# alexfrom0815/IR-BPP

Measured on AMD Instinct MI355X. Metric: env steps/sec (placements/sec) across N parallel bins, higher is better.
Workload: dtype f64

## Files before the change

include/irbpp.h:

```cpp
#ifndef IRBPP_H
#define IRBPP_H

#include <stdint.h>

#ifdef __cplusplus
extern "C" {
#endif

typedef struct irbpp_env irbpp_env;

typedef enum {
    IRBPP_OK = 0,
    IRBPP_ERR_ARG = -1,
    IRBPP_ERR_HIP = -2,
    IRBPP_ERR_STATE = -3,
    IRBPP_ERR_DEVICE = -4,
    IRBPP_ERR_NOMEM = -5
} irbpp_status;

typedef struct {
    int32_t num_bins;
    int32_t n_rot;
    int32_t selected;
    int32_t buffer_size;
// ... 13 lines not shown

#define IRBPP_TUNE_NO_BLOCK_PATH  1
#define IRBPP_TUNE_WIDE_KERNEL    2
#define IRBPP_TUNE_NARROW_KERNEL  4
#define IRBPP_TUNE_NO_BOX_PATH    8
#define IRBPP_TUNE_NO_ITEM_ORDER 16
#define IRBPP_TUNE_TRACE_CPW64   32
#define IRBPP_TUNE_TRACE_CPW32   64
#define IRBPP_TUNE_TRACE_CPW16  128
#define IRBPP_TUNE_INLINE_POLYGON 256
#define IRBPP_TUNE_NO_HEAVY_FIRST 512
#define IRBPP_TUNE_FUSED_APPLY 2048
#define IRBPP_TUNE_SPLIT_APPLY 4096
#define IRBPP_TUNE_BLOCK_EMIT 8192
#define IRBPP_TUNE_WAVE_EMIT 16384
#define IRBPP_TUNE_GRAPH 32768
#define IRBPP_TUNE_WG512 65536
#define IRBPP_TUNE_NO_WG512 131072
#define IRBPP_TUNE_TRACE_REFILL 262144
#define IRBPP_TUNE_NO_MIXED_PATH 524288
#define IRBPP_TUNE_CHAIN 1048576
#define IRBPP_TUNE_WG128 2097152
#define IRBPP_TUNE_RECT 4194304
#define IRBPP_TUNE_NO_SPECIALISED 1024

typedef struct {
    double*  reward_dev;
    uint8_t* done_dev;
    int32_t* counter_dev;
    double*  ratio_dev;
    double*  ep_reward_dev;
    int32_t* ep_len_dev;
    uint8_t* stable_dev;
    int32_t* err_dev;
} irbpp_step_out;

const char* irbpp_status_string(int status);
int irbpp_version(void);
const char* irbpp_source_hash(void);

int irbpp_create(const irbpp_config* cfg, irbpp_env** out);
int irbpp_destroy(irbpp_env* env);

int irbpp_load_shapes(irbpp_env* env, int32_t n_shapes,
                      const double* extents, const double* volumes,
                      const int32_t* dims, const int64_t* offsets, int64_t pool_len,
// ... 143 lines not shown
```

irbpp_amd/_lib.py:

```python
from __future__ import annotations

import ctypes as C
import os

from .build import LIB_PATH

c_i32_p = C.POINTER(C.c_int32)
c_f64_p = C.POINTER(C.c_double)


class IrbppConfig(C.Structure):
    _fields_ = [
        ("num_bins", C.c_int32), ("n_rot", C.c_int32), ("selected", C.c_int32), ("buffer_size", C.c_int32),
        ("resolution_a", C.c_double), ("resolution_h", C.c_double), ("resolution_z", C.c_double),
        ("bin", C.c_double * 3), ("scale_z", C.c_double),
        ("traj_start", C.c_int32), ("global_offset", C.c_int32), ("global_bins", C.c_int32),
        ("device", C.c_int32), ("stability", C.c_int32), ("tuning", C.c_int32), ("item_stream", C.c_int32),
    ]


TUNE_NO_BLOCK_PATH, TUNE_WIDE_KERNEL, TUNE_NARROW_KERNEL, TUNE_NO_BOX_PATH, TUNE_NO_ITEM_ORDER = 1, 2, 4, 8, 16
TUNE_TRACE_CPW64, TUNE_TRACE_CPW32, TUNE_TRACE_CPW16, TUNE_INLINE_POLYGON, TUNE_NO_HEAVY_FIRST = 32, 64, 128, 256, 512
TUNE_NO_SPECIALISED, TUNE_FUSED_APPLY, TUNE_SPLIT_APPLY, TUNE_BLOCK_EMIT, TUNE_WAVE_EMIT = 1024, 2048, 4096, 8192, 16384
TUNE_GRAPH, TUNE_WG512, TUNE_NO_WG512, TUNE_TRACE_REFILL, TUNE_NO_MIXED_PATH = 32768, 65536, 131072, 262144, 524288
TUNE_CHAIN, TUNE_WG128, TUNE_RECT = 1048576, 2097152, 4194304


class IrbppReplayView(C.Structure):
    _fields_ = [("states_dev", C.c_void_p), ("actions_dev", C.c_void_p), ("rewards_dev", C.c_void_p),
                ("nonterminals_dev", C.c_void_p), ("tree_dev", C.c_void_p), ("index_dev", C.c_void_p),
                ("full_dev", C.c_void_p), ("scaling_dev", C.c_void_p),
                ("n_env", C.c_int32), ("capacity", C.c_int32), ("obs_len", C.c_int32), ("n_step", C.c_int32)]


class IrbppReplayStore(C.Structure):
    _fields_ = [("states_dev", C.c_void_p), ("actions_dev", C.c_void_p), ("rewards_dev", C.c_void_p),
                ("nonterminals_dev", C.c_void_p), ("timesteps_dev", C.c_void_p), ("tree_dev", C.c_void_p),
                ("max_dev", C.c_void_p), ("index_dev", C.c_void_p), ("full_dev", C.c_void_p), ("t_dev", C.c_void_p),
                ("n_env", C.c_int32), ("capacity", C.c_int32), ("obs_len", C.c_int32)]


class IrbppEpisodeWindow(C.Structure):
    _fields_ = [("ring_dev", C.c_void_p), ("snapshot_dev", C.c_void_p), ("rows_dev", C.c_void_p), ("state_dev", C.c_void_p),
                ("window", C.c_int32), ("history", C.c_int32)]


class IrbppStepOut(C.Structure):
    _fields_ = [("reward_dev", C.c_void_p), ("done_dev", C.c_void_p), ("counter_dev", C.c_void_p),
# ... 120 lines not shown
```

irbpp_amd/build.py:

```python
from __future__ import annotations

import os
import shutil
import subprocess

PKG_DIR = os.path.dirname(os.path.abspath(__file__))
CSRC = os.path.join(PKG_DIR, "csrc")
LIB_PATH = os.path.join(PKG_DIR, "libirbpp_hip.so")
SOURCES = ["irbpp_capi.hip", "irbpp_kernels.hip", "irbpp_wide.hip", "irbpp_replay.hip", "irbpp_metrics.hip", "irbpp_metrics.h", "irbpp_device.h", "contours_device.h", "irbpp_itemgen.h",
           "irbpp_itemgen.hip", "irbpp_itemgen_device.h",
           os.path.join("..", "..", "include", "irbpp.h")]
HIPCC_FLAGS = ["--offload-arch=gfx950", "-O3", "-std=c++17", "-ffp-contract=off", "-fno-honor-nans",
               "-shared", "-fPIC", "-Wno-unused-value"]


def source_hash() -> str:
    import hashlib
    h = hashlib.sha256(" ".join(HIPCC_FLAGS).encode())
    for name in sorted(SOURCES):
        with open(os.path.join(CSRC, name), "rb") as f:
            h.update(f.read())
    return h.hexdigest()[:16]


def _hipcc() -> str:
    for cand in (shutil.which("hipcc"), "/opt/rocm/bin/hipcc"):
        if cand and os.path.exists(cand):
            return cand
    raise RuntimeError("hipcc not found: the HIP library cannot be built on this machine")


def built_hash(path: str = LIB_PATH) -> str:
    try:
# ... 36 lines not shown
```

irbpp_amd/csrc/irbpp_capi.hip:

```cpp
#include <hip/hip_runtime.h>
#include <math.h>
#include <stdint.h>
#include <stdio.h>
#include <stdlib.h>
#include <string.h>

#include <new>
#include <utility>
#include <vector>

#include "../../include/irbpp.h"
#include "irbpp_device.h"
#include "irbpp_kernels.hip"
#include "irbpp_wide.hip"
#include "irbpp_replay.hip"
#include "irbpp_itemgen.hip"
#include "irbpp_metrics.hip"
#include "irbpp_itemgen.h"

using namespace irbpp;

struct irbpp_env {
    irbpp_config cfg;
    Params P;
    Tables T;
    State S;
    bool shapes_loaded = false, seq_loaded = false, was_reset = false;
    bool item_order = false;
    long long* phase_cycles = nullptr;
    int32_t* auto_actions = nullptr;
    int heavy_turn = 0;
    int32_t* err_mirror = nullptr;
    std::vector<std::pair<const float*, int32_t*>> obs_buffers;
    std::vector<hipEvent_t> timing;
    size_t timing_next = 0, timing_used = 0;
// ... 338 lines not shown
            if (block_b && ((block_rots >> r) & 1))
                for (int ti = 0; ti < s.fx / block_b; ++ti)
                    for (int tj = 0; tj < s.fy / block_b; ++tj) {
                        const int64_t e0 = off + (int64_t)(ti * block_b) * s.fy + tj * block_b;
                        if (mask_bottom[e0] != 0.0)
                            blkcell.push_back(Cell{height_bottom[e0], (ti * block_b / P.step) * mb_w + tj * block_b / P.step, 0});
                    }
            s.nblk = (int32_t)blkcell.size() - s.oblk;
            if (!box && (!block_b || mixed))
                for (int e = 0; e < s.nb; ++e) {
                    const Cell& c = bcell[s.ob + e];
                    const int ci = c.ij & 0xFFFF, cj = c.ij >> 16;
                    const int off = ((ci % P.step) * P.step + cj % P.step) * P.AC + (ci / P.step) * P.Ay + cj / P.step;
                    gcell.push_back(GCell{c.v, off * 8, 0});
                }
            if (box) {
                while (s.bx < s.fx && mask_bottom[off + (int64_t)s.bx * s.fy] != 0.0) ++s.bx;
                while (s.by < s.fy && mask_bottom[off + s.by] != 0.0) ++s.by;
                s.bc = height_bottom[off];
            }
            if (s.nb == 0 && !s.has_out) return IRBPP_ERR_ARG;
        }
    }
    if (bcell.empty()) bcell.push_back(Cell{0.0, 0, 0});
    if (tcell.empty()) tcell.push_back(Cell{0.0, 0, 0});
    if (blkcell.empty()) blkcell.push_back(Cell{0.0, 0, 0});
    if (gcell.empty()) gcell.push_back(GCell{0.0, 0, 0});
    for (int i = 0; i < 8; ++i) gcell.push_back(GCell{0.0, 0, 0});
    Tables& T = env->T;
    int rc = dev_upload(env, &T.sr, sr.data(), sr.size());
    if (rc == IRBPP_OK) rc = dev_upload(env, &T.bcell, (const Cell*)bcell.data(), bcell.size());
    if (rc == IRBPP_OK) rc = dev_upload(env, &T.tcell, (const Cell*)tcell.data(), tcell.size());
    if (rc == IRBPP_OK) rc = dev_upload(env, &T.blkcell, (const Cell*)blkcell.data(), blkcell.size());
    if (rc == IRBPP_OK) rc = dev_upload(env, &T.gcell, (const GCell*)gcell.data(), gcell.size());
    if (rc == IRBPP_OK) rc = dev_upload(env, &T.volume, volumes, (size_t)n_shapes);
    if (rc != IRBPP_OK) return rc;
    T.n_shapes = n_shapes;
    if (block_b || box) {
        env->P.block_b = block_b;
        env->P.block_rots = block_rots;
        env->P.mb_h = mb_h;
        env->P.mb_w = mb_w;
        env->P.box = box ? 1 : 0;
        layout_lds_host(env->P);
        if (env->P.lds_bytes_full > 160 * 1024) return IRBPP_ERR_ARG;
        if (raise_lds_limits() != IRBPP_OK) return IRBPP_ERR_HIP;
// ... 773 lines not shown
```

irbpp_amd/csrc/irbpp_device.h:

```cpp
#pragma once
#include <hip/hip_runtime.h>
#include <stdint.h>

namespace irbpp {

#ifndef IRBPP_CONTOUR_IPT
#define IRBPP_CONTOUR_IPT 2
#endif
constexpr int CONTOUR_IPT = IRBPP_CONTOUR_IPT;

constexpr int WMETA = 8;
constexpr int NXCD = 8;
constexpr int XCD_STRIDE = 64;
#ifndef IRBPP_TRACE_P
#define IRBPP_TRACE_P 2
#endif
constexpr int ROUND_POINTS = 64 * IRBPP_TRACE_P, ROUND_BYTES = ROUND_POINTS * 7;
constexpr int MAX_BINS = 1 << 20;
constexpr int TUNED_MAX_LEVELS = 31;
constexpr int MAX_LEVELS = 222;

struct ShapeRot {
    int32_t fx, fy;
    int32_t ax, ay;
    int32_t nb, nt;
    int32_t ob, ot;
    int32_t has_out;
    int32_t pad;
    int32_t nblk, oblk;
    int32_t bx, by;
    double bc;
    double ext_x, ext_y, ext_z;
    double ext_z_r;
    double com_x, com_y;
};

struct Cell {
    double v;
    int32_t ij;
    int32_t pad;
};

struct alignas(16) GCell { double b; int32_t off; int32_t pad; };

struct Tables {
    const ShapeRot* sr;
    const Cell* bcell;
    const Cell* tcell;
    const Cell* blkcell;
    const GCell* gcell;
    const double* volume;
// ... 246 lines not shown
```

irbpp_amd/csrc/irbpp_kernels.hip:

```cpp
#include <hip/hip_runtime.h>
#include <math.h>
#include <stdint.h>

#include "contours_device.h"
#include "irbpp_device.h"
#include "../../include/irbpp.h"

#ifndef IRBPP_PASS
#define IRBPP_PASS 1
#endif

#undef IRBPP_HERE
#undef IRBPP_PASS_NS
#if IRBPP_PASS == 1
#define IRBPP_HERE ::irbpp::
#elif IRBPP_PASS == 2
#define IRBPP_HERE ::irbpp::wg512::
#define IRBPP_PASS_NS wg512
#else
#define IRBPP_HERE ::irbpp::wg128::
#define IRBPP_PASS_NS wg128
#endif

namespace irbpp {
// ... 244 lines not shown
};

__device__ inline Lds carve_lds(unsigned char* smem, const Params& P) {
    Lds L;
    L.sr = (int*)(smem + P.o_sr);
    L.hm = (double*)(smem + P.o_hm);
    L.mb = (double*)(smem + P.o_mb);
    L.c2 = (double*)(smem + P.o_c2);
    L.m1 = (double*)(smem + P.o_m1);
    L.posz = (double*)(smem + P.o_posz);
    L.lev = smem + P.o_lev;
    L.present = (unsigned long long*)(smem + P.o_present);
    L.taskidx = (uint16_t*)(smem + P.o_taskidx);
    L.tasklist = (uint16_t*)(smem + P.o_tasklist);
    L.img = (uint16_t*)(smem + P.o_img);
    L.clist = (uint16_t*)(smem + P.o_clist);
    L.dps = (uint32_t*)(smem + P.o_dps);
    L.vmask = (uint32_t*)(smem + P.o_vmask);
    L.vbits = (uint32_t*)(smem + P.o_vbits);
    L.scratch = smem + P.o_scratch;
    L.redd = (double*)(smem + P.o_red);
    L.redi = (int*)(L.redd + 8);
    return L;
}

#endif
constexpr int CONTOUR_IMGS = CONTOUR_IPT * (BLOCK / 16);
constexpr int CONTOUR_CLIST = 256;

__device__ inline int contour_tasks(const Params& P, const Lds& L) {
    const int tid = threadIdx.x, R = P.R;
    int ntasks = 0;
    for (int r = 0; r < R; ++r) ntasks += __popcll(L.present[r]);
#pragma unroll 1
    for (int t = tid; t < R * 64; t += BLOCK) {
        const int r = t >> 6, l = t & 63;
        const unsigned long long m = L.present[r];
        if ((m >> l) & 1ull) {
            int base = 0;
            for (int q = 0; q < r; ++q) base += __popcll(L.present[q]);
            const int idx = base + __popcll(m & ((1ull << l) - 1ull));
            L.tasklist[idx] = (uint16_t)((r << 8) | l);
            L.taskidx[t] = (uint16_t)idx;
        }
    }
    return ntasks;
// ... 440 lines not shown
            const int pi = fdiv(t, P.mb_w, P.mg_mbw), pj = t - pi * P.mb_w;
            const double* c = L.c2 + pi * Ay + pj;
            double m = -1e300;
            for (int i = 0; i < mq; ++i)
                for (int j = 0; j < mq; ++j) m = fmax(m, c[i * Ay + j]);
            L.mb[t] = m;
        }
    }
    __syncthreads();
    const bool bl_lds = use_block && item >= 0 && bl_total <= AC / 2;
    typedef int32_t bl_words __attribute__((ext_vector_type(4)));
    bl_words* const bl = (bl_words*)L.c2;
    if (bl_lds) {
        if (tid < bl_total) {
            bl_words w;
            w.x = __double2loint(bl_entry.v); w.y = __double2hiint(bl_entry.v); w.z = bl_entry.ij * 8; w.w = 0;
            bl[tid] = w;
        }
        __syncthreads();
    }

    const int lane = tid & 63, wave = __builtin_amdgcn_readfirstlane(tid >> 6);
    int my_valid = 0;
    if (use_block || use_box) {
    constexpr int CELLS = BLOCK >= 256 ? 1 : 256 / BLOCK;
    if (CELLS > 1 && use_box) __builtin_trap();
#pragma unroll 1
    for (int ci = 0; ci < CELLS; ++ci) {
    const int cell = CELLS == 1 ? tid : tid + ci * BLOCK;
    const int X = fdiv(cell, Ay, P.mg_ay), Y = cell - X * Ay;
    double zs[8];
    bool vs[8];
    if (use_box) {
        double* const m1 = L.m1;
#pragma unroll
        for (int r = 0; r < 8; ++r) {
            zs[r] = 1e3;
            vs[r] = false;
            if (r >= R || item < 0) continue;
            const ShapeRot* sp = (const ShapeRot*)srw + r;
            const int s_ax = __builtin_amdgcn_readfirstlane(sp->ax), s_ay = __builtin_amdgcn_readfirstlane(sp->ay);
            const int bx = __builtin_amdgcn_readfirstlane(sp->bx), by = __builtin_amdgcn_readfirstlane(sp->by);
            const int has_out = __builtin_amdgcn_readfirstlane(sp->has_out);
            const double ext_z_r = sp->ext_z_r, bc = sp->bc;
            for (int idx = tid; idx < P.Hx * Ay; idx += BLOCK) {
                const int i = fdiv(idx, Ay, P.mg_ay), yy = idx - i * Ay;
                if (yy <= Ay - s_ay) {
                    const double* rowp = L.hm + tile_row_part(P, i);
                    double m = -1e300;
                    for (int j = 0; j < by; ++j) m = fmax(m, rowp[tile_col_part(P, yy * P.step + j)]);
                    m1[idx] = m;
                }
            }
            __syncthreads();
            const bool in_range = cell < AC && X <= Ax - s_ax && Y <= Ay - s_ay;
            if (in_range) {
                const double* colp = m1 + X * P.step * Ay + Y;
                double m = -1e300;
                for (int i = 0; i < bx; ++i) m = fmax(m, colp[i * Ay]);
                m = m - bc;
                if (has_out) m = fmax(m, 0.0);
                zs[r] = m;
                vs[r] = round6_scaled(m + ext_z_r - P.bin_z) <= 0.0;
            }
            __syncthreads();
        }
    } else {
    int ncell_next = 0, off_next = 0;
    Cell pre = {};
    if (bl_lds) {
    for (int rep = 0; rep < IRBPP_REPS(2); ++rep) {
#pragma unroll
    for (int r = 0; r < 8; ++r) {
        zs[r] = 1e3;
        vs[r] = false;
        if (r >= R || !((brots >> r) & 1u)) continue;
        const ShapeRot* sp = (const ShapeRot*)srw + r;
        const int s_ax = __builtin_amdgcn_readfirstlane(sp->ax), s_ay = __builtin_amdgcn_readfirstlane(sp->ay);
        const int has_out = __builtin_amdgcn_readfirstlane(sp->has_out);
        const int ne = __builtin_amdgcn_readfirstlane(sp->nblk), e0 = __builtin_amdgcn_readfirstlane(sp->oblk) - bl_first;
        const double ext_z_r = sp->ext_z_r;
        const bool in_range = cell < AC && X <= Ax - s_ax && Y <= Ay - s_ay;
        if (in_range) {
            const char* const hb = (const char*)(L.mb + X * P.mb_w + Y);
            const bl_words* const be = bl + e0;
            double m = has_out ? 0.0 : -1e300;
            int u = 0;
            for (; u + 4 <= ne; u += 4) {
                bl_words q[4];
                double hv[4];
#pragma unroll
                for (int k = 0; k < 4; ++k) q[k] = be[u + k];
#pragma unroll
                for (int k = 0; k < 4; ++k) hv[k] = *(const double*)(hb + q[k].z);
#pragma unroll
                for (int k = 0; k < 4; ++k) m = fmax(m, hv[k] - __hiloint2double(q[k].y, q[k].x));
            }
            for (; u < ne; ++u) {
                const bl_words q = be[u];
// ... 2 lines not shown
            zs[r] = m;
            vs[r] = round6_scaled(m + ext_z_r - P.bin_z) <= 0.0;
        }
    }
    }
    } else
    for (int rep = 0; rep < IRBPP_REPS(2); ++rep) {
    if (item >= 0) {
        const ShapeRot* s0 = (const ShapeRot*)srw;
        ncell_next = __builtin_amdgcn_readfirstlane(s0->nblk);
        off_next = __builtin_amdgcn_readfirstlane(s0->oblk);
        const Cell* c0 = T.blkcell + off_next;
        if (ncell_next > 0) pre = c0[lane < ncell_next ? lane : ncell_next - 1];
    }
#pragma unroll
    for (int r = 0; r < 8; ++r) {
        zs[r] = 1e3;
        vs[r] = false;
        if (r >= R || item < 0) continue;
        const ShapeRot* sp = (const ShapeRot*)srw + r;
        const int s_ax = __builtin_amdgcn_readfirstlane(sp->ax), s_ay = __builtin_amdgcn_readfirstlane(sp->ay);
        const int has_out = __builtin_amdgcn_readfirstlane(sp->has_out);
        const double ext_z_r = sp->ext_z_r;
        const int ncell = ((brots >> r) & 1u) ? ncell_next : 0, off0 = off_next;
        Cell c = pre;
        if (r + 1 < R) {
            const ShapeRot* sn = sp + 1;
            ncell_next = __builtin_amdgcn_readfirstlane(sn->nblk);
            off_next = __builtin_amdgcn_readfirstlane(sn->oblk);
            const Cell* cn = T.blkcell + off_next;
            if (ncell_next > 0) pre = cn[lane < ncell_next ? lane : ncell_next - 1];
        }
        const bool in_range = cell < AC && X <= Ax - s_ax && Y <= Ay - s_ay;
        const double* h0 = L.mb + X * P.mb_w + Y;
        double m = has_out ? 0.0 : -1e300;
        const Cell* cells = T.blkcell + off0;
        for (int base = 0; base < ncell; base += 64) {
            if (base > 0) {
                const int idx = base + lane < ncell ? base + lane : ncell - 1;
                c = cells[idx];
            }
            const int cnt = ncell - base < 64 ? ncell - base : 64;
            int c_off = c.ij;
            int c_lo = (int)__double2loint(c.v), c_hi = (int)__double2hiint(c.v);
            asm volatile("" : "+v"(c_off), "+v"(c_lo), "+v"(c_hi));
            if (in_range) {
                int u = 0;
                for (; u + 8 <= cnt; u += 8) {
                    double hv[8], vv[8];
#pragma unroll
                    for (int k = 0; k < 8; ++k) {
                        const int off = __builtin_amdgcn_readlane(c_off, u + k);
                        vv[k] = __hiloint2double(__builtin_amdgcn_readlane(c_hi, u + k),
                                                 __builtin_amdgcn_readlane(c_lo, u + k));
                        hv[k] = h0[off];
                    }
#pragma unroll
                    for (int k = 0; k < 8; ++k) m = fmax(m, hv[k] - vv[k]);
                }
                for (; u < cnt; ++u) {
                    const int off = __builtin_amdgcn_readlane(c_off, u);
                    const double v = __hiloint2double(__builtin_amdgcn_readlane(c_hi, u),
                                                      __builtin_amdgcn_readlane(c_lo, u));
                    m = fmax(m, h0[off] - v);
                }
            }
        }
        if (in_range && ((brots >> r) & 1u)) {
            zs[r] = m;
            vs[r] = round6_scaled(m + ext_z_r - P.bin_z) <= 0.0;
        }
    }
    }
    }
    int level_code[8];
    for (int rep = 0; rep < IRBPP_REPS(7); ++rep) {
    if (rep) my_valid = 0;
    const bool rows_align = (1 << P.g_ysh) == Ay;
#pragma unroll
    for (int r = 0; r < 8; ++r) {
        level_code[r] = 255;
        if (r >= R || (!use_box && !((brots >> r) & 1u))) continue;
        const double z = zs[r];
        const bool valid = vs[r];
        if (cell < AC) {
            if (debug_out) {
                const KernArgsPtr ka = cold_args();
                ka->io.posz_out[((size_t)b * R + r) * AC + cell] = z;
                ka->io.mask_out[((size_t)b * R + r) * AC + cell] = valid ? 1 : 0;
            }
            int code = 255;
            if (valid) {
                if (!debug_out) zdst[r * AC + cell] = z;
                const int li = np_floor_divide_int(z, P.res_z, P.inv_res_z);
                if (li != -1) {
                    const int idx = li + 32;
                    if (idx < 0 || idx > 63) raise_error(S, IRBPP_DEVERR_LEVEL_RANGE);
                    else code = idx;
                }
                ++my_valid;
                L.lev[r * AC + cell] = (uint8_t)code;
                if (!rows_align) atomicOr(&L.vbits[r * 16 + X], 1u << Y);
            }
            level_code[r] = code;
        }
        if (rows_align) {
            const unsigned long long bal = __ballot(valid && cell < AC);
            if (Y == 0 && cell < AC) L.vbits[r * 16 + X] = (uint32_t)(bal >> (lane & ~(Ay - 1))) & ((1u << Ay) - 1u);
        }
    }
#pragma unroll
    for (int r = 0; r < 8; ++r) {
        if (r >= R || (!use_box && !((brots >> r) & 1u))) continue;
        const int code = level_code[r];
        unsigned long long todo = __ballot(code != 255), bits = 0ull;
        while (todo) {
            const int c = __builtin_amdgcn_readlane(code, __ffsll((long long)todo) - 1);
            bits |= 1ull << c;
            todo &= ~__ballot(code == c);
        }
        if ((tid & 63) == 0 && bits) atomicOr(&L.present[r], bits);
    }
    }
    }
    }
    if (use_lists) {
    const int ysh = P.g_ysh, rpw = 64 >> ysh;
    const int rs = lane >> ysh, Y = lane & ((1 << ysh) - 1);
    const bool rows_whole = (1 << ysh) == Ay;
    int my_grp = 0;
    if (lane < R && item >= 0 && !((brots >> lane) & 1u)) {
        const ShapeRot* sp = (const ShapeRot*)srw + lane;
        const int wx = Ax - sp->ax + 1, wy = Ay - sp->ay + 1;
        if (wx > 0 && wy > 0) my_grp = (wx + rpw - 1) >> (6 - ysh);
    }
    const int t3 = my_grp > 3 ? 2 : (my_grp > 0 ? 1 : 0), t2 = (my_grp + 1) >> 1;
// ... 91 lines not shown
            const char* h2[2] = {h1[0], lane_base(X0 + rpw)};
            const char* h3[3] = {h1[0], h2[1], lane_base(X0 + 2 * rpw)};
            if (G == 1) gcell_walk<1, 0>(gc, nb, h1, init, (double(&)[1])z[0]);
            else if (G == 2) gcell_walk<2, 0>(gc, nb, h2, init, (double(&)[2])z[0]);
            else gcell_walk<3, 0>(gc, nb, h3, init, z);
        }
        task_finish(r, X0, s_ax, s_ay, ext_z_r, z[0]);
        if (G > 1) task_finish(r, X0 + rpw, s_ax, s_ay, ext_z_r, z[1]);
        if (G > 2) task_finish(r, X0 + 2 * rpw, s_ax, s_ay, ext_z_r, z[2]);
        task_presence(r);
    }
    asm volatile("" :: "v"(pref));
    if (debug_out)
        for (int i = tid; i < R * AC; i += BLOCK) {
            const int r = fdiv(i, AC, P.mg_ac), cell = i - r * AC, X = fdiv(cell, Ay, P.mg_ay), Y = cell - X * Ay;
            const ShapeRot* sp = (const ShapeRot*)srw + r;
            if (((brots >> r) & 1u) == 0u && (item < 0 || X > Ax - sp->ax || Y > Ay - sp->ay)) {
                const KernArgsPtr ka = cold_args();
                ka->io.posz_out[((size_t)b * R + r) * AC + cell] = 1e3;
                ka->io.mask_out[((size_t)b * R + r) * AC + cell] = 0;
            }
        }
    }
    return block_sum_int(my_valid, L.redi);
}

__device__ inline void emit_observation(const Params& P, const State& S, const StepIO& io, const Lds& L, int b, int item,
                                        int nvalid, float* obs, const double* zsrc, const uint32_t* gvalid);
template <int IPT>
__device__ inline void split_handover(const Params& P, const State& S, const Lds& L, int b, int slot, int item, int nvalid);

template <int PATH, bool CHAIN = false>
__device__ inline void observe_location(const Params& P, const Tables& T, const State& S, const StepIO& io,
                                        const Lds& L, int b, int item, float* obs, bool debug_out, bool sr_staged,
                                        unsigned char* chain_lds = nullptr) {
    item = __builtin_amdgcn_readfirstlane(item);
    const int tid = threadIdx.x;
    const int R = P.R, AC = P.AC, Ax = P.Ax, Ay = P.Ay;
    const int X = fdiv(tid, Ay, P.mg_ay), Y = tid - X * Ay;
    const int nvalid = IRBPP_HERE overlap_test<PATH>(P, T, S, io, L, b, item, debug_out, S.w_posz + (size_t)b * R * AC, sr_staged, false);
    if (debug_out) return;
    if (tid < 9) obs[5 * P.S + tid] = tid == 0 ? (float)item : 0.0f;
    for (int rep = 0; rep < IRBPP_REPS(8); ++rep)
    for (TileWalk w = IRBPP_HERE tile_walk_begin(P, tid); w.lin < P.Hc; tile_walk_next(w)) obs[5 * P.S + 9 + w.lin] = (float)L.hm[tile_walk_index(P, w)];
    __syncthreads();
    stamp(io, b, 2);

    if (io.phase_cycles && tid == 0)
        for (int k = 5; k < PHASE_ROW; ++k)
            if (k < 8 || k > 10) io.phase_cycles[(size_t)b * PHASE_ROW + k] = 0;
    if constexpr (CHAIN) {
        {
            uint32_t* gb = S.w_valid + (size_t)b * P.R * 16;
#pragma unroll 1
            for (int i = tid; i < P.R * 16; i += BLOCK) gb[i] = L.vbits[i];
        }
        __syncthreads();
        ::irbpp::contour_stage(P, S, L, nullptr);
        __builtin_amdgcn_fence(__ATOMIC_RELEASE, "workgroup");
        __syncthreads();
        __builtin_amdgcn_fence(__ATOMIC_ACQUIRE, "workgroup");
        Lds Le = L;
        Le.img = (uint16_t*)chain_lds;
        ::irbpp::emit_observation(P, S, io, Le, b, item, nvalid, obs, S.w_posz + (size_t)b * R * AC, S.w_valid + (size_t)b * R * 16);
        return;
    }
    IRBPP_HERE split_handover<(CONTOUR_IPT * 256) / BLOCK>(P, S, L, b, (int)blockIdx.x + io.block_off, item, nvalid);
    if (io.phase_cycles && tid == 0)
        io.phase_cycles[(size_t)b * PHASE_ROW + 5] = (long long)clock64() - io.phase_cycles[(size_t)b * PHASE_ROW + 2];
}

#if IRBPP_PASS == 1
__device__ __forceinline__ unsigned long long sortable_f64(double v) {
    const unsigned long long b = (unsigned long long)__double_as_longlong(v);
    return (b >> 63) ? ~b : (b | 0x8000000000000000ull);
}
constexpr int SEL_PER_THREAD = (8 * 256 + BLOCK - 1) / BLOCK;

template <typename KEY>
__device__ inline void select_smallest(const Params& P, const Lds& L, const double* zsrc, const uint32_t* vbits, int n, int want,
                                       const KEY& key, uint32_t* out, uint32_t* sel, uint32_t* hist) {
    const int tid = threadIdx.x;
    auto value = [&](uint32_t k) {
        const uint32_t r = k >> 16, x = (k >> 8) & 255u, y = k & 255u;
        if (vbits != nullptr && !((vbits[r * 16 + x] >> y) & 1u)) return 1e3;
        return zsrc[r * P.AC + x * P.Ay + y];
    };
// ... 81 lines not shown
                const int i = ((t >> sh) << (sh + 1)) | (t & (j - 1)), l = i | j;
                const uint32_t ah = khi[i], al = klo[i], bh = khi[l], bl = klo[l];
                const uint32_t ap = kps[i], bp = kps[l];
                const bool a_gt_b = ah > bh || (ah == bh && (al > bl || (al == bl && ap > bp)));
                if (a_gt_b == ((i & k) == 0)) {
                    khi[i] = bh; klo[i] = bl; kps[i] = (uint16_t)bp;
                    khi[l] = ah; klo[l] = al; kps[l] = (uint16_t)ap;
                }
            }
            const int j_next = j > 1 ? (j >> 1) : k;
            if (j >= 128 || j_next >= 128 || (j == 1 && k == npad)) __syncthreads();
            else IRBPP_WAVE_SYNC();
        }
    for (int r = tid; r < want; r += BLOCK) out[r] = sel[kps[r]];
    __syncthreads();
}

#ifdef IRBPP_AB_EMIT_ACCOUNT
#define IRBPP_EMIT_STAMP(k) do { if (io.phase_cycles && threadIdx.x == 0) io.phase_cycles[(size_t)b * PHASE_ROW + (k)] = (long long)clock64(); } while (0)
#else
#define IRBPP_EMIT_STAMP(k) do {} while (0)
#endif
__device__ inline void emit_observation(const Params& P, const State& S, const StepIO& io, const Lds& L, int b, int item,
                                        int nvalid, float* obs, const double* zsrc, const uint32_t* gvalid) {
    const int tid = threadIdx.x;
    const int R = P.R, AC = P.AC, Ax = P.Ax, Ay = P.Ay;
    const int X = fdiv(tid, Ay, P.mg_ay), Y = tid - X * Ay;
    const int prev_rows = io.obs_rows != nullptr ? io.obs_rows[b] : -1;
    if (tid == 0) ((unsigned long long*)L.redd)[7] = ~0ull;
    uint32_t* keys = (uint32_t*)L.scratch;
    uint32_t* okey = keys + R * AC;
    uint32_t* hist = (uint32_t*)L.img;
    int n = 0;
    if (tid < 64) {
        const int lane = tid, cx = lane & 15;
        for (int r0 = 0; r0 < R; r0 += 4) {
            const int r = r0 + (lane >> 4);
            uint32_t col = 0u;
            if (r < R && cx < Ay) {
#pragma unroll
                for (int cy = 0; cy < 16; ++cy) col |= ((L.vmask[r * 16 + cy] >> cx) & 1u) << cy;
                col &= (1u << Ax) - 1u;
            }
            const int cnt = __popc(col), incl = wave_inclusive_sum(cnt);
            int at = n + incl - cnt;
            while (col != 0u) {
                const int cy = __ffs((int)col) - 1;
                col &= col - 1u;
                keys[at++] = ((uint32_t)r << 16) | ((uint32_t)cy << 8) | (uint32_t)cx;
            }
            n += __builtin_amdgcn_readlane(incl, 63);
        }
        if (tid == 0) L.redi[34] = n;
    }
    __syncthreads();
    n = L.redi[34];
    IRBPP_EMIT_STAMP(11);
    int nrows;
    bool fallback = false;
    const uint32_t* rows;
    if (n > 0 && n <= P.S) {
        nrows = n;
        rows = keys;
    } else if (n > P.S) {
// ... 139 lines not shown
            __syncthreads();
            if (L.redi[11] >= 0) {
                uint2* flat = ka->S.w_cand + (size_t)L.redi[12] * P.seg_cap + L.redi[11];
#pragma unroll 1
                for (int i = tid; i < total; i += BLOCK) {
                    const uint32_t e = clist[i];
                    flat[i] = make_uint2((uint32_t)b, ((uint32_t)(base + (e & 127u)) << 8) | (((e >> 11) & 15u) << 4) | ((e >> 7) & 15u));
                }
            }
            ncand += total;
        }
        __syncthreads();
    }
    uint32_t* gv = ka->S.w_vmask + (size_t)b * P.R * 16;
    for (int rep = 0; rep < IRBPP_REPS(14); ++rep)
#pragma unroll 1
    for (int i = tid; i < P.R * 16; i += BLOCK) gv[i] = L.vmask[i];
    if (tid == 0) {
        int32_t* m = ka->S.w_meta + (size_t)b * WMETA;
        m[0] = ntasks;
        m[1] = ncand;
        m[2] = nvalid;
        m[3] = item;
        int heavy = 0;
        const int turn = ka->io.heavy_turn;
        if (turn >= 0 && ncand + niso >= P.heavy_thr) {
            int32_t* hv = ka->S.w_heavy + (size_t)turn * (XCD_STRIDE + P.heavy_cap);
            const int pos = atomicAdd(hv, 1);
            if (pos < P.heavy_cap) { hv[XCD_STRIDE + pos] = b; heavy = 1; }
        }
        m[4] = heavy;
    }
}

#if IRBPP_PASS == 1
template <bool HEAVY_FIRST, int SPEC>
__device__ __forceinline__ void emit_body(const Params& P_run, const Tables& T, const State& S, const StepIO& io, const int mode, unsigned char* smem) {
    Params P_spec;
    const Params& P = SPEC == 0 ? P_run : (P_spec = specialise<SPEC>(P_run), P_spec);
    Lds L = {};
    L.vmask = (uint32_t*)(smem + P.e_vmask);
    L.redd = (double*)(smem + P.e_red);
    L.redi = (int*)(L.redd + 8);
    L.img = (uint16_t*)(smem + P.e_hist);
    L.scratch = smem + P.e_keys;
    const bool some = mode == MODE_RESET && io.bin_list != nullptr;
// ... 14 lines not shown
            cnt = cnt < P.heavy_cap ? cnt : P.heavy_cap;
            if ((int)blockIdx.x >= cnt) return;
            b = hv[XCD_STRIDE + blockIdx.x];
            slot = b;
            mapped = true;
        } else {
            slot -= hg;
        }
    }
    if (!mapped) {
        b = ((mode == MODE_STEP || mode == MODE_CANDS) && io.use_order) ? S.order[slot] : some ? io.bin_list[slot] : slot;
        if constexpr (HEAVY_FIRST)
            if (io.heavy_turn >= 0 && b >= 0 && b < P.N && S.w_meta[(size_t)b * WMETA + 4] != 0) return;
    }
    if (b < 0 || b >= P.N) return;
#ifdef IRBPP_AB_EMIT_ACCOUNT
    if (io.phase_cycles && tid == 0) { io.phase_cycles[(size_t)b * PHASE_ROW + 6] = t_entry; io.phase_cycles[(size_t)b * PHASE_ROW + 7] = (long long)clock64(); }
#endif
    float* obs = io.obs + (size_t)(some ? slot : b) * io.obs_stride;
    const uint32_t* gv = S.w_vmask + (size_t)b * P.R * 16;
#pragma unroll 1
    for (int i = tid; i < P.R * 16; i += BLOCK) L.vmask[i] = gv[i];
    const int nvalid = S.w_meta[(size_t)b * WMETA + 2], item = S.w_meta[(size_t)b * WMETA + 3];
    __syncthreads();
    stamp(io, b, 3);
    emit_observation(P, S, io, L, b, item, nvalid, obs, S.w_posz + (size_t)b * P.R * P.AC, S.w_valid + (size_t)b * P.R * 16);
    IRBPP_EMIT_STAMP(14);
}
#define IRBPP_EMIT_KERNEL(NAME, HF, SPEC)                                                                                \
    extern "C" __global__ void __launch_bounds__(BLOCK) __attribute__((amdgpu_waves_per_eu(8, 8)))                      \
    NAME(const Params P, const Tables T, const State S, const StepIO io, const int mode) {                              \
        extern __shared__ __attribute__((aligned(16))) unsigned char smem[];                                            \
        emit_body<HF, SPEC>(P, T, S, io, mode, smem);                                                                   \
    }
IRBPP_EMIT_KERNEL(irbpp_emit_kernel, true, 0)
#ifndef IRBPP_NO_SPEC
IRBPP_EMIT_KERNEL(irbpp_emit_kernel_s1, true, 1)
IRBPP_EMIT_KERNEL(irbpp_emit_kernel_s2, true, 2)
IRBPP_EMIT_KERNEL(irbpp_emit_kernel_s3, true, 3)
IRBPP_EMIT_KERNEL(irbpp_emit_kernel_s4, true, 4)
IRBPP_EMIT_KERNEL(irbpp_emit_kernel_s5, true, 5)
#endif

template <int SPEC>
__device__ __forceinline__ void emit_wave_body(const Params& P_run, const Tables& T, const State& S, const StepIO& io, const int mode,
                                               unsigned char* smem) {
    Params P_spec;
    const Params& P = SPEC == 0 ? P_run : (P_spec = specialise<SPEC>(P_run), P_spec);
    int* const need = (int*)(smem + P.e_need);
    const int tid = threadIdx.x, lane = tid & 63, wave = __builtin_amdgcn_readfirstlane(tid >> 6);
    const int R = P.R, AC = P.AC, Ax = P.Ax, Ay = P.Ay;
    const bool some = mode == MODE_RESET && io.bin_list != nullptr;
    if (blockIdx.x == 0 && tid < NXCD) { S.w_total[tid * XCD_STRIDE] = 0; S.w_nround[tid * XCD_STRIDE] = 0; }
    if (blockIdx.x == 0 && tid == 0 && io.err_out != nullptr) *io.err_out = *S.err;
    const int local = (int)blockIdx.x * WAVES + wave;
    const int slot = local + io.block_off;
    int b = -1;
    if (local < io.n_slots) b = ((mode == MODE_STEP || mode == MODE_CANDS) && io.use_order) ? S.order[slot] : some ? io.bin_list[slot] : slot;
    if (b >= P.N) b = -1;
    b = __builtin_amdgcn_readfirstlane(b);
    if (lane == 0) need[wave] = -1;
    if (b >= 0) {
        uint32_t* const vm = (uint32_t*)(smem + wave * P.ew_bytes);
        uint32_t* const keys = vm + R * 16;
        const uint32_t* gv = S.w_vmask + (size_t)b * R * 16;
        for (int i = lane; i < R * 16; i += 64) vm[i] = gv[i];
        const int nvalid = S.w_meta[(size_t)b * WMETA + 2], item = S.w_meta[(size_t)b * WMETA + 3];
        const int prev_rows = io.obs_rows != nullptr ? io.obs_rows[b] : -1;
        float* const obs = io.obs + (size_t)(some ? slot : b) * io.obs_stride;
        const double* const zsrc = S.w_posz + (size_t)b * R * AC;
        const uint32_t* const gvalid = S.w_valid + (size_t)b * R * 16;
        stamp(io, b, 3, lane == 0);
        IRBPP_WAVE_SYNC();
        const int cx = lane & 15;
        auto column = [&](int r) {
            uint32_t col = 0u;
            if (r < R && cx < Ay) {
#pragma unroll
                for (int cy = 0; cy < 16; ++cy) col |= ((vm[r * 16 + cy] >> cx) & 1u) << cy;
                col &= (1u << Ax) - 1u;
            }
            return col;
        };
        int n = 0;
#pragma unroll 1
        for (int r0 = 0; r0 < R; r0 += 4) n += __builtin_amdgcn_readlane(wave_inclusive_sum(__popc(column(r0 + (lane >> 4)))), 63);
        if (n > P.S || (n == 0 && nvalid > 0)) {
            if (lane == 0) need[wave] = b;
        } else {
            int at0 = 0;
#pragma unroll 1
            for (int r0 = 0; r0 < R; r0 += 4) {
                const int r = r0 + (lane >> 4);
                uint32_t col = column(r);
                const int cnt = __popc(col), incl = wave_inclusive_sum(cnt);
                int at = at0 + incl - cnt;
                while (col != 0u) {
                    const int cy = __ffs((int)col) - 1;
                    col &= col - 1u;
                    keys[at++] = ((uint32_t)r << 16) | ((uint32_t)cy << 8) | (uint32_t)cx;
                }
                at0 += __builtin_amdgcn_readlane(incl, 63);
// ... 52 lines not shown
            }
            stamp(io, b, 4, lane == 0);
        }
    }
    __syncthreads();
    if ((need[0] & need[1] & need[2] & need[3]) == -1) return;
    Lds L = {};
    L.vmask = (uint32_t*)(smem + P.e_vmask);
    L.redd = (double*)(smem + P.e_red);
    L.redi = (int*)(L.redd + 8);
    L.img = (uint16_t*)(smem + P.e_hist);
    L.scratch = smem + P.e_keys;
#pragma unroll 1
    for (int w = 0; w < WAVES; ++w) {
        const int bw = __builtin_amdgcn_readfirstlane(need[w]);
        if (bw < 0) continue;
        const int slot_w = (int)blockIdx.x * WAVES + w + io.block_off;
        float* const obs = io.obs + (size_t)(some ? slot_w : bw) * io.obs_stride;
        const uint32_t* gv = S.w_vmask + (size_t)bw * R * 16;
        __syncthreads();
#pragma unroll 1
        for (int i = tid; i < R * 16; i += BLOCK) L.vmask[i] = gv[i];
        const int nvalid = S.w_meta[(size_t)bw * WMETA + 2], item = S.w_meta[(size_t)bw * WMETA + 3];
        __syncthreads();
        stamp(io, bw, 3);
        emit_observation(P, S, io, L, bw, item, nvalid, obs, S.w_posz + (size_t)bw * R * AC, S.w_valid + (size_t)bw * R * 16);
    }
}
#define IRBPP_EMIT_WAVE_KERNEL(NAME, SPEC)                                                                                  \
    extern "C" __global__ void __launch_bounds__(BLOCK) __attribute__((amdgpu_waves_per_eu(8, 8)))                      \
    NAME(const Params P, const Tables T, const State S, const StepIO io, const int mode) {                              \
        extern __shared__ __attribute__((aligned(16))) unsigned char smem[];                                            \
        emit_wave_body<SPEC>(P, T, S, io, mode, smem);                                                                  \
    }
IRBPP_EMIT_WAVE_KERNEL(irbpp_emit_wave_kernel, 0)
#ifndef IRBPP_NO_SPEC
IRBPP_EMIT_WAVE_KERNEL(irbpp_emit_wave_kernel_s1, 1)
IRBPP_EMIT_WAVE_KERNEL(irbpp_emit_wave_kernel_s2, 2)
IRBPP_EMIT_WAVE_KERNEL(irbpp_emit_wave_kernel_s5, 5)
#endif

#ifndef IRBPP_TRACE_SHORT
#define IRBPP_TRACE_SHORT 0
#endif
constexpr int TRACE_P = IRBPP_TRACE_P;
constexpr int TRACE_CAP = 128;
constexpr int TRACE_LDS_CAP = 56, TRACE_SLOT = TRACE_LDS_CAP + 4;
constexpr int TRACE_SPILL = TRACE_CAP - TRACE_LDS_CAP;
constexpr int TRACE_SHORT = IRBPP_TRACE_SHORT;
// ... 1395 lines not shown
```

Before: 64.08 million.

## Alias rotations with identical footprints to skip redundant placement evaluation

At shape load time, the host detects rotations of each item whose footprint, bottom mask and heights are bit-identical to an earlier rotation and records an alias index in the previously unused pad field of ShapeRot. The step kernels then copy z/valid results from the aliased rotation instead of recomputing them, skip level coding and contour work for aliased rotations, and the emit paths read the vmask row through a packed alias map stored in w_meta. This is meant to remove duplicated per-rotation height-map scans for symmetric items, at the cost of extra branching, a readfirstlane per rotation and a new metadata slot. It can be turned off with a tuning flag and is disabled for wide mode or more than eight rotations.

```diff
diff --git a/include/irbpp.h b/include/irbpp.h
--- a/include/irbpp.h
+++ b/include/irbpp.h
@@ -59,6 +59,7 @@
 #define IRBPP_TUNE_CHAIN 1048576
 #define IRBPP_TUNE_WG128 2097152
 #define IRBPP_TUNE_RECT 4194304
+#define IRBPP_TUNE_NO_ROT_ALIAS 8388608
 #define IRBPP_TUNE_NO_SPECIALISED 1024
 
 typedef struct {
diff --git a/irbpp_amd/_lib.py b/irbpp_amd/_lib.py
--- a/irbpp_amd/_lib.py
+++ b/irbpp_amd/_lib.py
@@ -23,7 +23,7 @@
 TUNE_TRACE_CPW64, TUNE_TRACE_CPW32, TUNE_TRACE_CPW16, TUNE_INLINE_POLYGON, TUNE_NO_HEAVY_FIRST = 32, 64, 128, 256, 512
 TUNE_NO_SPECIALISED, TUNE_FUSED_APPLY, TUNE_SPLIT_APPLY, TUNE_BLOCK_EMIT, TUNE_WAVE_EMIT = 1024, 2048, 4096, 8192, 16384
 TUNE_GRAPH, TUNE_WG512, TUNE_NO_WG512, TUNE_TRACE_REFILL, TUNE_NO_MIXED_PATH = 32768, 65536, 131072, 262144, 524288
-TUNE_CHAIN, TUNE_WG128, TUNE_RECT = 1048576, 2097152, 4194304
+TUNE_CHAIN, TUNE_WG128, TUNE_RECT, TUNE_NO_ROT_ALIAS = 1048576, 2097152, 4194304, 8388608
 
 
 class IrbppReplayView(C.Structure):
diff --git a/irbpp_amd/build.py b/irbpp_amd/build.py
--- a/irbpp_amd/build.py
+++ b/irbpp_amd/build.py
@@ -8,7 +8,7 @@
 CSRC = os.path.join(PKG_DIR, "csrc")
 LIB_PATH = os.path.join(PKG_DIR, "libirbpp_hip.so")
 SOURCES = ["irbpp_capi.hip", "irbpp_kernels.hip", "irbpp_wide.hip", "irbpp_replay.hip", "irbpp_metrics.hip", "irbpp_metrics.h", "irbpp_device.h", "contours_device.h", "irbpp_itemgen.h",
-           "irbpp_itemgen.hip", "irbpp_itemgen_device.h",
+           "irbpp_itemgen.hip", "irbpp_itemgen_device.h", "irbpp_rotalias.h",
            os.path.join("..", "..", "include", "irbpp.h")]
 HIPCC_FLAGS = ["--offload-arch=gfx950", "-O3", "-std=c++17", "-ffp-contract=off", "-fno-honor-nans",
                "-shared", "-fPIC", "-Wno-unused-value"]
diff --git a/irbpp_amd/csrc/irbpp_capi.hip b/irbpp_amd/csrc/irbpp_capi.hip
--- a/irbpp_amd/csrc/irbpp_capi.hip
+++ b/irbpp_amd/csrc/irbpp_capi.hip
@@ -11,6 +11,7 @@
 
 #include "../../include/irbpp.h"
 #include "irbpp_device.h"
+#include "irbpp_rotalias.h"
 #include "irbpp_kernels.hip"
 #include "irbpp_wide.hip"
 #include "irbpp_replay.hip"
@@ -395,6 +396,23 @@
             if (s.nb == 0 && !s.has_out) return IRBPP_ERR_ARG;
         }
     }
+    {
+        const bool off = P.wide || (env->cfg.tuning & IRBPP_TUNE_NO_ROT_ALIAS) || R > 8;
+        std::vector<RotView> views((size_t)R);
+        std::vector<int32_t> alias((size_t)R);
+        for (int k = 0; k < n_shapes; ++k) {
+            for (int r = 0; r < R; ++r) {
+                const size_t i = (size_t)k * R + r;
+                views[r] = RotView{sr[i].fx, sr[i].fy, sr[i].ax, sr[i].ay, sr[i].has_out, sr[i].ext_z_r, mask_bottom + offsets[i], height_bottom + offsets[i]};
+            }
+            rot_aliases(views.data(), R, alias.data());
+            for (int r = 0; r < R; ++r) {
+                const int c = alias[r];
+                const bool skips = box || (((block_rots >> r) & 1) && ((block_rots >> c) & 1));
+                sr[(size_t)k * R + r].alias = (off || !skips) ? r : c;
+            }
+        }
+    }
     if (bcell.empty()) bcell.push_back(Cell{0.0, 0, 0});
     if (tcell.empty()) tcell.push_back(Cell{0.0, 0, 0});
     if (blkcell.empty()) blkcell.push_back(Cell{0.0, 0, 0});
diff --git a/irbpp_amd/csrc/irbpp_device.h b/irbpp_amd/csrc/irbpp_device.h
--- a/irbpp_amd/csrc/irbpp_device.h
+++ b/irbpp_amd/csrc/irbpp_device.h
@@ -26,7 +26,7 @@
     int32_t nb, nt;
     int32_t ob, ot;
     int32_t has_out;
-    int32_t pad;
+    int32_t alias;
     int32_t nblk, oblk;
     int32_t bx, by;
     double bc;
diff --git a/irbpp_amd/csrc/irbpp_kernels.hip b/irbpp_amd/csrc/irbpp_kernels.hip
--- a/irbpp_amd/csrc/irbpp_kernels.hip
+++ b/irbpp_amd/csrc/irbpp_kernels.hip
@@ -290,6 +290,17 @@
     L.redd = (double*)(smem + P.o_red);
     L.redi = (int*)(L.redd + 8);
     return L;
+}
+
+constexpr uint32_t ALIAS_IDENTITY = 0x76543210u;
+__device__ __forceinline__ uint32_t alias_map(const Lds& L, int R, int item) {
+    if (item < 0) return ALIAS_IDENTITY;
+    const ShapeRot* sa = (const ShapeRot*)L.sr;
+    uint32_t m = ALIAS_IDENTITY;
+#pragma unroll
+    for (int r = 1; r < 8; ++r)
+        if (r < R) m = (m & ~(15u << (4 * r))) | ((uint32_t)sa[r].alias << (4 * r));
+    return m;
 }
 
 #endif
@@ -776,6 +787,10 @@
 
     const int lane = tid & 63, wave = __builtin_amdgcn_readfirstlane(tid >> 6);
     int my_valid = 0;
+#define IRBPP_ALIAS_OF(r) __builtin_amdgcn_readfirstlane(((const ShapeRot*)srw)[r].alias)
+#define IRBPP_ALIAS_COPY(r, al)                                                                                         \
+    _Pragma("unroll") for (int c_ = 0; c_ < 7; ++c_)                                                                    \
+        if (c_ < (r) && (al) == c_) { zs[r] = zs[c_]; vs[r] = vs[c_]; }
     if (use_block || use_box) {
     constexpr int CELLS = BLOCK >= 256 ? 1 : 256 / BLOCK;
     if (CELLS > 1 && use_box) __builtin_trap();
@@ -793,6 +808,7 @@
             vs[r] = false;
             if (r >= R || item < 0) continue;
             const ShapeRot* sp = (const ShapeRot*)srw + r;
+            if (const int al = IRBPP_ALIAS_OF(r); al != r) { IRBPP_ALIAS_COPY(r, al) continue; }
             const int s_ax = __builtin_amdgcn_readfirstlane(sp->ax), s_ay = __builtin_amdgcn_readfirstlane(sp->ay);
             const int bx = __builtin_amdgcn_readfirstlane(sp->bx), by = __builtin_amdgcn_readfirstlane(sp->by);
             const int has_out = __builtin_amdgcn_readfirstlane(sp->has_out);
@@ -829,6 +845,7 @@
         zs[r] = 1e3;
         vs[r] = false;
         if (r >= R || !((brots >> r) & 1u)) continue;
+        if (const int al = IRBPP_ALIAS_OF(r); al != r) { IRBPP_ALIAS_COPY(r, al) continue; }
         const ShapeRot* sp = (const ShapeRot*)srw + r;
         const int s_ax = __builtin_amdgcn_readfirstlane(sp->ax), s_ay = __builtin_amdgcn_readfirstlane(sp->ay);
         const int has_out = __builtin_amdgcn_readfirstlane(sp->has_out);
@@ -877,7 +894,9 @@
         const int s_ax = __builtin_amdgcn_readfirstlane(sp->ax), s_ay = __builtin_amdgcn_readfirstlane(sp->ay);
         const int has_out = __builtin_amdgcn_readfirstlane(sp->has_out);
         const double ext_z_r = sp->ext_z_r;
-        const int ncell = ((brots >> r) & 1u) ? ncell_next : 0, off0 = off_next;
+        const int al = IRBPP_ALIAS_OF(r);
+        const bool own = al == r;
+        const int ncell = (((brots >> r) & 1u) && own) ? ncell_next : 0, off0 = off_next;
         Cell c = pre;
         if (r + 1 < R) {
             const ShapeRot* sn = sp + 1;
@@ -921,7 +940,9 @@
                 }
             }
         }
-        if (in_range && ((brots >> r) & 1u)) {
+        if (!own) {
+            IRBPP_ALIAS_COPY(r, al)
+        } else if (in_range && ((brots >> r) & 1u)) {
             zs[r] = m;
             vs[r] = round6_scaled(m + ext_z_r - P.bin_z) <= 0.0;
         }
@@ -947,12 +968,14 @@
             int code = 255;
             if (valid) {
                 if (!debug_out) zdst[r * AC + cell] = z;
+                if (IRBPP_ALIAS_OF(r) == r) {
                 const int li = np_floor_divide_int(z, P.res_z, P.inv_res_z);
                 if (li != -1) {
                     const int idx = li + 32;
                     if (idx < 0 || idx > 63) raise_error(S, IRBPP_DEVERR_LEVEL_RANGE);
                     else code = idx;
                 }
+                }
                 ++my_valid;
                 L.lev[r * AC + cell] = (uint8_t)code;
                 if (!rows_align) atomicOr(&L.vbits[r * 16 + X], 1u << Y);
@@ -966,7 +989,7 @@
     }
 #pragma unroll
     for (int r = 0; r < 8; ++r) {
-        if (r >= R || (!use_box && !((brots >> r) & 1u))) continue;
+        if (r >= R || (!use_box && !((brots >> r) & 1u)) || IRBPP_ALIAS_OF(r) != r) continue;
         const int code = level_code[r];
         unsigned long long todo = __ballot(code != 255), bits = 0ull;
         while (todo) {
@@ -1104,11 +1127,13 @@
             }
         }
     }
+#undef IRBPP_ALIAS_COPY
+#undef IRBPP_ALIAS_OF
     return block_sum_int(my_valid, L.redi);
 }
 
 __device__ inline void emit_observation(const Params& P, const State& S, const StepIO& io, const Lds& L, int b, int item,
-                                        int nvalid, float* obs, const double* zsrc, const uint32_t* gvalid);
+                                        int nvalid, float* obs, const double* zsrc, const uint32_t* gvalid, uint32_t amap);
 template <int IPT>
 __device__ inline void split_handover(const Params& P, const State& S, const Lds& L, int b, int slot, int item, int nvalid);
 
@@ -1144,7 +1169,8 @@
         __builtin_amdgcn_fence(__ATOMIC_ACQUIRE, "workgroup");
         Lds Le = L;
         Le.img = (uint16_t*)chain_lds;
-        ::irbpp::emit_observation(P, S, io, Le, b, item, nvalid, obs, S.w_posz + (size_t)b * R * AC, S.w_valid + (size_t)b * R * 16);
+        ::irbpp::emit_observation(P, S, io, Le, b, item, nvalid, obs, S.w_posz + (size_t)b * R * AC, S.w_valid + (size_t)b * R * 16,
+                                  ::irbpp::alias_map(L, R, item));
         return;
     }
     IRBPP_HERE split_handover<(CONTOUR_IPT * 256) / BLOCK>(P, S, L, b, (int)blockIdx.x + io.block_off, item, nvalid);
@@ -1272,7 +1298,7 @@
 #define IRBPP_EMIT_STAMP(k) do {} while (0)
 #endif
 __device__ inline void emit_observation(const Params& P, const State& S, const StepIO& io, const Lds& L, int b, int item,
-                                        int nvalid, float* obs, const double* zsrc, const uint32_t* gvalid) {
+                                        int nvalid, float* obs, const double* zsrc, const uint32_t* gvalid, uint32_t amap) {
     const int tid = threadIdx.x;
     const int R = P.R, AC = P.AC, Ax = P.Ax, Ay = P.Ay;
     const int X = fdiv(tid, Ay, P.mg_ay), Y = tid - X * Ay;
@@ -1288,8 +1314,9 @@
             const int r = r0 + (lane >> 4);
             uint32_t col = 0u;
             if (r < R && cx < Ay) {
-#pragma unroll
-                for (int cy = 0; cy < 16; ++cy) col |= ((L.vmask[r * 16 + cy] >> cx) & 1u) << cy;
+                const uint32_t* const vrow = L.vmask + ((amap >> (4 * r)) & 15u) * 16;
+#pragma unroll
+                for (int cy = 0; cy < 16; ++cy) col |= ((vrow[cy] >> cx) & 1u) << cy;
                 col &= (1u << Ax) - 1u;
             }
             const int cnt = __popc(col), incl = wave_inclusive_sum(cnt);
@@ -1475,6 +1502,7 @@
         m[1] = ncand;
         m[2] = nvalid;
         m[3] = item;
+        m[5] = (int32_t)alias_map(L, P.R, item);
         int heavy = 0;
         const int turn = ka->io.heavy_turn;
         if (turn >= 0 && ncand + niso >= P.heavy_thr) {
@@ -1535,9 +1563,10 @@
 #pragma unroll 1
     for (int i = tid; i < P.R * 16; i += BLOCK) L.vmask[i] = gv[i];
     const int nvalid = S.w_meta[(size_t)b * WMETA + 2], item = S.w_meta[(size_t)b * WMETA + 3];
+    const uint32_t amap = (uint32_t)S.w_meta[(size_t)b * WMETA + 5];
     __syncthreads();
     stamp(io, b, 3);
-    emit_observation(P, S, io, L, b, item, nvalid, obs, S.w_posz + (size_t)b * P.R * P.AC, S.w_valid + (size_t)b * P.R * 16);
+    emit_observation(P, S, io, L, b, item, nvalid, obs, S.w_posz + (size_t)b * P.R * P.AC, S.w_valid + (size_t)b * P.R * 16, amap);
     IRBPP_EMIT_STAMP(14);
 }
 #define IRBPP_EMIT_KERNEL(NAME, HF, SPEC)                                                                                \
@@ -1579,6 +1608,7 @@
         const uint32_t* gv = S.w_vmask + (size_t)b * R * 16;
         for (int i = lane; i < R * 16; i += 64) vm[i] = gv[i];
         const int nvalid = S.w_meta[(size_t)b * WMETA + 2], item = S.w_meta[(size_t)b * WMETA + 3];
+        const uint32_t amap = (uint32_t)S.w_meta[(size_t)b * WMETA + 5];
         const int prev_rows = io.obs_rows != nullptr ? io.obs_rows[b] : -1;
         float* const obs = io.obs + (size_t)(some ? slot : b) * io.obs_stride;
         const double* const zsrc = S.w_posz + (size_t)b * R * AC;
@@ -1589,8 +1619,9 @@
         auto column = [&](int r) {
             uint32_t col = 0u;
             if (r < R && cx < Ay) {
-#pragma unroll
-                for (int cy = 0; cy < 16; ++cy) col |= ((vm[r * 16 + cy] >> cx) & 1u) << cy;
+                const uint32_t* const vrow = vm + ((amap >> (4 * r)) & 15u) * 16;
+#pragma unroll
+                for (int cy = 0; cy < 16; ++cy) col |= ((vrow[cy] >> cx) & 1u) << cy;
                 col &= (1u << Ax) - 1u;
             }
             return col;
@@ -1689,9 +1720,10 @@
 #pragma unroll 1
         for (int i = tid; i < R * 16; i += BLOCK) L.vmask[i] = gv[i];
         const int nvalid = S.w_meta[(size_t)bw * WMETA + 2], item = S.w_meta[(size_t)bw * WMETA + 3];
+        const uint32_t amap_w = (uint32_t)S.w_meta[(size_t)bw * WMETA + 5];
         __syncthreads();
         stamp(io, bw, 3);
-        emit_observation(P, S, io, L, bw, item, nvalid, obs, S.w_posz + (size_t)bw * R * AC, S.w_valid + (size_t)bw * R * 16);
+        emit_observation(P, S, io, L, bw, item, nvalid, obs, S.w_posz + (size_t)bw * R * AC, S.w_valid + (size_t)bw * R * 16, amap_w);
     }
 }
 #define IRBPP_EMIT_WAVE_KERNEL(NAME, SPEC)                                                                                  \
diff --git a/irbpp_amd/csrc/irbpp_rotalias.h b/irbpp_amd/csrc/irbpp_rotalias.h
--- /dev/null
+++ b/irbpp_amd/csrc/irbpp_rotalias.h
@@ -0,0 +1,43 @@
+#pragma once
+#include <stdint.h>
+#include <string.h>
+
+namespace irbpp {
+
+struct RotView {
+    int32_t fx, fy;
+    int32_t ax, ay;
+    int32_t has_out;
+    double ext_z_r;
+    const double* mask_bottom;
+    const double* height_bottom;
+};
+
+inline bool rot_same_bits(double a, double b) {
+    uint64_t ua, ub;
+    memcpy(&ua, &a, 8);
+    memcpy(&ub, &b, 8);
+    return ua == ub;
+}
+
+inline bool rot_same_observation(const RotView& a, const RotView& b) {
+    if (a.fx != b.fx || a.fy != b.fy || a.ax != b.ax || a.ay != b.ay || a.has_out != b.has_out) return false;
+    if (!rot_same_bits(a.ext_z_r, b.ext_z_r)) return false;
+    const int64_t n = (int64_t)a.fx * a.fy;
+    for (int64_t e = 0; e < n; ++e) {
+        const bool in_a = a.mask_bottom[e] != 0.0, in_b = b.mask_bottom[e] != 0.0;
+        if (in_a != in_b) return false;
+        if (in_a && !rot_same_bits(a.height_bottom[e], b.height_bottom[e])) return false;
+    }
+    return true;
+}
+
+inline void rot_aliases(const RotView* rots, int R, int32_t* alias) {
+    for (int r = 0; r < R; ++r) {
+        alias[r] = r;
+        for (int c = 0; c < r; ++c)
+            if (alias[c] == c && rot_same_observation(rots[c], rots[r])) { alias[r] = c; break; }
+    }
+}
+
+}
```

After: 69.45 million, median of 6. 1.08x the previous value.
